# showlab/EgoVLP

Measured on AMD Instinct MI355X. Metric: clip-pairs/sec (whole node), 4f/224^2 ViT-B + 32-tok text, B=32/GPU, train step (fwd+gather+EgoNCE+bwd+AdamW), higher is better.
Workload: dtype fp16 (every Linear and both attentions of the video blocks, forward and backward) + bf16 (patch embedding, text tower, heads) MFMA operands, fp32 accumulate

## Files before the change

egovlp_amd/csrc/block.hip:

```cpp
#include <hip/hip_runtime.h>

#include <algorithm>

#include "layer_call.h"

namespace {

struct FwdLayout {
  int64_t n3_hi, n3_lo, mean3, rstd3, qkvt_hi, qkvt_lo, at_hi, at_lo, lse_t, work_t;
  int64_t tr, n1_hi, n1_lo, mean1, rstd1, qkvs_hi, qkvs_lo, as_hi, as_lo, lse_s, work_s;
  int64_t sr, n2_hi, n2_lo, mean2, rstd2, h_hi, h_lo, z;
  int64_t n3_bf, n1_bf, n2_bf, h_bf;
  int64_t n1c, mean1c, rstd1c, qc, oc, n2c, hc;
  int64_t total;
};

struct Geo {
  int64_t M, S, D, Hd;
  int P, Pb;
};

inline bool is_train(const egv_block_geom& g) { return (g.train & 1) != 0; }
inline bool is_tail(const egv_block_geom& g) { return (g.train & 2) != 0; }

// ... 277 lines not shown
  if (!gp || !pp || !iop || !geom_ok(*gp) || !(gp->train & 1)) return EGV_ERR_ARG;
  const egv_block_geom& g = *gp;
  const egv_block_params& p = *pp;
  const egv_block_bwd_io& io = *iop;
  if (!io.g_out || !io.x || !io.fwd_arena || !io.bwd_arena || !io.d_x || !io.dx_hi || !io.grads) return EGV_ERR_ARG;
  const bool tail = is_tail(g);
  if (tail && io.g_hi) return EGV_ERR_ARG;
  const Geo o = geo_of(g);
  const int Pb = o.Pb;
  const FwdLayout F = fwd_layout(g);
  const BwdLayout L = bwd_layout(g, io.wgrad_ksplit);
  int64_t goff[18], gtot;
  grad_layout(g, goff, gtot);
  const int32_t M = (int32_t)o.M, D = (int32_t)o.D, Hd = (int32_t)o.Hd;
  for (int i = 0; i < (tail ? 3 : 6); ++i)
    if (!p.wt_hi[i] || (Pb == 3 && !p.wt_lo[i])) return EGV_ERR_ARG;
  if (Pb == 3 && (!io.dx_lo || (io.g_hi && !io.g_lo))) return EGV_ERR_ARG;
  const bool h16 = Pb == 4;
  constexpr float A1_INV = 1.0f / (1.0f - 0.015625f);
  const char* FA = (const char*)io.fwd_arena;
  char* A = (char*)io.bwd_arena;
  hipStream_t main_s = (hipStream_t)stream;
  const bool x2 = o.P == 2 && !h16;
  const egv_bf16 *n3_hi, *n3_lo, *at_hi, *at_lo, *n1_hi, *n1_lo, *as_hi, *as_lo, *n2_hi, *n2_lo, *h_hi, *h_lo, *qt_hi, *qt_lo, *qs_hi, *qs_lo;
  saved_planes(FA, Pb, x2 ? F.n3_bf : F.n3_hi, F.n3_lo, n3_hi, n3_lo);
  saved_planes(FA, Pb, F.at_hi, F.at_lo, at_hi, at_lo);
  saved_planes(FA, Pb, x2 ? F.n1_bf : F.n1_hi, F.n1_lo, n1_hi, n1_lo);
  saved_planes(FA, Pb, F.as_hi, F.as_lo, as_hi, as_lo);
  saved_planes(FA, Pb, x2 ? F.n2_bf : F.n2_hi, F.n2_lo, n2_hi, n2_lo);
  saved_planes(FA, Pb, x2 ? F.h_bf : F.h_hi, F.h_lo, h_hi, h_lo);
  saved_planes(FA, Pb, F.qkvt_hi, F.qkvt_lo, qt_hi, qt_lo);
  saved_planes(FA, Pb, F.qkvs_hi, F.qkvs_lo, qs_hi, qs_lo);
  const bool proj1 = (g.f16_single & 8) != 0;
  const egv_bf16 *as_lo_f = (proj1 || h16) ? nullptr : at<egv_bf16>(FA, F.as_lo), *at_lo_f = (proj1 || h16) ? nullptr : at<egv_bf16>(FA, F.at_lo);
  const int afmt = h16 ? (proj1 ? 3 : 2) : (proj1 ? 1 : 0);
  const int amode = (afmt << 1) | (h16 ? 8 | 16 : 0);
  const float walpha[6] = {h16 && !(g.f16_single & 4) ? A1_INV : 1.0f, h16 && !proj1 ? A1_INV : 1.0f, h16 && !(g.f16_single & 4) ? A1_INV : 1.0f,
                           h16 && !proj1 ? A1_INV : 1.0f, h16 && !(g.f16_single & 1) ? A1_INV : 1.0f, h16 && !(g.f16_single & 2) ? A1_INV : 1.0f};
  const int Pg = Pb;
  const float *tr = at<float>(FA, F.tr), *sr = at<float>(FA, F.sr);
  float* grads = io.grads;

  bool defer_reduce = true;
  for (int i = 1; i < 6; ++i) defer_reduce = defer_reduce && io.side_stream[i] == io.side_stream[0];
#ifdef EGV_NO_MULTI_REDUCE
  defer_reduce = false;
#endif
  auto wgrad = [&](int i, const egv_bf16* dy_hi, const egv_bf16* dy_lo, int64_t lddy, const egv_bf16* x_hi, const egv_bf16* x_lo,
                   int64_t ldx, int64_t row0 = 0, int64_t rows = 0) -> int {
    int64_t N, K;
    wshape(o, i, N, K);
    if (rows) N = rows;
    hipStream_t s = main_s;
    if (io.side_stream[i]) {
      s = (hipStream_t)io.side_stream[i];
      if (hipEventRecord((hipEvent_t)io.side_event[i], main_s) != hipSuccess) return EGV_ERR_LAUNCH;
      if (hipStreamWaitEvent(s, (hipEvent_t)io.side_event[i], 0) != hipSuccess) return EGV_ERR_LAUNCH;
    }
    egv_gemm_desc d = tn_desc(dy_hi, dy_lo, lddy, x_hi, x_lo, ldx, N, K, M, Pg, grads + goff[i] + row0 * K, grads + goff[6 + i] + row0, io.wgrad_ksplit[i],
                              at<float>(A, L.partial[i]), g.grid_cap);
    d.alpha = walpha[i];
    if (defer_reduce && d.ksplit > 1) d.accumulate = 2;
    return egv_gemm_nt(&d, s);
  };

  auto ln_in = [&](egv_gemm_desc& d, float* buf) {
    if (h16) { d.out_hi = (egv_bf16*)buf; d.ldoh = D; d.out_fmt = 4; }
    else { d.out_f32 = buf; d.ldo = D; }
  };
  const int ln_fmt = h16 ? 3 : 0;
  float* d_sr = at<float>(A, L.d_sr);
  float* d_n1 = at<float>(A, L.d_n1);
  if (tail) {
    const float *w_q = (const float*)p.w_hi[2], *w_proj = (const float*)p.w_hi[3], *w_fc1 = (const float*)p.w_hi[4],
                *w_fc2 = (const float*)p.w_hi[5];
    if (!w_q || !w_proj || !w_fc1 || !w_fc2) return EGV_ERR_ARG;
    const int32_t B = g.B;
    const int64_t ldc = o.S * o.D;
    const float* G = io.g_out;
    const float *n1c = at<float>(FA, F.n1c), *qc = at<float>(FA, F.qc), *oc = at<float>(FA, F.oc), *n2c = at<float>(FA, F.n2c),
                *hc = at<float>(FA, F.hc);
    float *dzc = at<float>(A, L.dzc), *dn2c = at<float>(A, L.dn2c), *dsrc = at<float>(A, L.dsrc), *doc = at<float>(A, L.doc),
          *dqc = at<float>(A, L.dqc), *lw = at<float>(A, L.lin_work);
    EGV_TRY(egv_cls_linear_dgrad(G, D, w_fc2, Hd, B, D, Hd, at<float>(FA, F.z), dzc, Hd, 0, lw, stream));
    EGV_TRY(egv_cls_linear_wgrad(G, D, hc, Hd, B, D, Hd, grads + goff[5], Hd, grads + goff[11], stream));
    EGV_TRY(egv_cls_linear_dgrad(dzc, Hd, w_fc1, D, B, Hd, D, nullptr, dn2c, D, 0, lw, stream));
    EGV_TRY(egv_cls_linear_wgrad(dzc, Hd, n2c, D, B, Hd, D, grads + goff[4], D, grads + goff[10], stream));
    EGV_TRY(egv_layernorm_bwd_partial(dn2c, nullptr, nullptr, D, sr, D, p.n2w, at<float>(FA, F.mean2), at<float>(FA, F.rstd2), B, D, G, nullptr,
                                      dsrc, D, nullptr, nullptr, 0, grads + goff[16], grads + goff[17], at<float>(A, L.ln_work[0]), stream));
    EGV_TRY(egv_cls_linear_wgrad(dsrc, D, oc, D, B, D, D, grads + goff[3], D, grads + goff[9], stream));
    EGV_TRY(egv_cls_linear_dgrad(dsrc, D, w_proj, D, B, D, D, nullptr, doc, D, 0, lw, stream));
    uint16_t *dkv_hi = (uint16_t*)at<egv_bf16>(A, L.dqkvs_hi), *dkv_lo = (uint16_t*)at<egv_bf16>(A, L.dqkvs_lo);
    const uint16_t *kv_hi = (const uint16_t*)at<egv_bf16>(FA, F.qkvs_hi), *kv_lo = (const uint16_t*)at<egv_bf16>(FA, F.qkvs_lo);
    EGV_TRY(egv_cls_attn_bwd(qc, D, kv_hi, kv_lo, kv_hi + D, kv_lo ? kv_lo + D : nullptr, 2 * D, h16 ? 1 : 0, oc, doc, at<float>(FA, F.lse_s), B,
                             (int32_t)o.S, g.H, dqc, dkv_hi, dkv_lo, dkv_hi + D, dkv_lo ? dkv_lo + D : nullptr, 2 * D, h16 ? 1 : 0, stream));
    EGV_TRY(egv_cls_linear_wgrad(dqc, D, n1c, D, B, D, D, grads + goff[2], D, grads + goff[8], stream));
    EGV_TRY(wgrad(2, (const egv_bf16*)dkv_hi, (const egv_bf16*)dkv_lo, 2 * D, n1_hi, n1_lo, D, D, 2 * D));
    {
      egv_gemm_desc d = nt_desc((const egv_bf16*)dkv_hi, (const egv_bf16*)dkv_lo, 2 * D, p.wt_hi[2] + D, p.wt_lo[2] ? p.wt_lo[2] + D : nullptr,
                                p.ldwt[2], M, D, 2 * D, Pg, g.grid_cap);
      ln_in(d, d_n1);
      EGV_TRY(egv_gemm_nt(&d, stream));
    }
    EGV_TRY(egv_cls_linear_dgrad(dqc, D, w_q, D, B, D, D, nullptr, d_n1, ldc, h16 ? 2 : 1, lw, stream));
  } else {
    const egv_bf16 *g_hi = io.g_hi, *g_lo = Pb == 3 ? io.g_lo : nullptr;
    if (!g_hi) {
      egv_bf16 *gh = at<egv_bf16>(A, L.g_hi), *gl = at<egv_bf16>(A, L.g_lo);
      if (h16) EGV_TRY(egv_f16x2_encode(io.g_out, D, M, D, gh, nullptr, nullptr, D, 2, stream));
      else EGV_TRY(egv_split_f32(io.g_out, D, M, D, gh, gl, D, nullptr, nullptr, 0, nullptr, stream));
      g_hi = gh; g_lo = gl;
    }
    egv_bf16 *dz_hi = at<egv_bf16>(A, L.dz_hi), *dz_lo = at<egv_bf16>(A, L.dz_lo);
    {
      egv_gemm_desc d = nt_desc(g_hi, g_lo, D, p.wt_hi[5], p.wt_lo[5], p.ldwt[5], M, Hd, D, Pg, g.grid_cap);
      d.act = EGV_ACT_GELU_BWD; d.aux_in = at<float>(FA, F.z); d.ldaux = Hd; d.aux_bf16 = g.z_bf16 ? (h16 ? 3 : 2) : 0;
      d.out_hi = dz_hi; d.out_lo = dz_lo; d.ldoh = Hd;
      if (h16) d.out_fmt = 4;
      EGV_TRY(egv_gemm_nt(&d, stream));
    }
    EGV_TRY(wgrad(5, g_hi, g_lo, D, h_hi, h_lo, Hd));
    EGV_TRY(wgrad(4, dz_hi, dz_lo, Hd, n2_hi, n2_lo, D));
    float* d_n2 = at<float>(A, L.d_n2);
    {
      egv_gemm_desc d = nt_desc(dz_hi, dz_lo, Hd, p.wt_hi[4], p.wt_lo[4], p.ldwt[4], M, D, Hd, Pg, g.grid_cap);
      ln_in(d, d_n2);
      EGV_TRY(egv_gemm_nt(&d, stream));
    }
    egv_bf16 *dsr_hi = at<egv_bf16>(A, L.dsr_hi), *dsr_lo = at<egv_bf16>(A, L.dsr_lo);
    EGV_TRY(egv_layernorm_bwd_partial(h16 ? nullptr : d_n2, h16 ? (const egv_bf16*)d_n2 : nullptr, nullptr, D, sr, D, p.n2w, at<float>(FA, F.mean2),
                              at<float>(FA, F.rstd2), M, D, io.g_out, nullptr,
                              d_sr, D, dsr_hi, dsr_lo, ln_fmt, grads + goff[16], grads + goff[17], at<float>(A, L.ln_work[0]), stream));
    EGV_TRY(wgrad(3, dsr_hi, dsr_lo, D, as_hi, as_lo, D));
    egv_bf16 *das_hi = at<egv_bf16>(A, L.das_hi), *das_lo = at<egv_bf16>(A, L.das_lo);
    {
      egv_gemm_desc d = nt_desc(dsr_hi, dsr_lo, D, p.wt_hi[3], p.wt_lo[3], p.ldwt[3], M, D, D, Pg, g.grid_cap);
      d.out_hi = das_hi; d.out_lo = das_lo; d.ldoh = D;
      if (h16) d.out_fmt = 4;
      EGV_TRY(egv_gemm_nt(&d, stream));
    }
    egv_bf16 *dqs_hi = at<egv_bf16>(A, L.dqkvs_hi), *dqs_lo = at<egv_bf16>(A, L.dqkvs_lo);
    EGV_TRY(egv_divided_attn_bwd(qs_hi, qs_lo, as_hi, as_lo_f, das_hi, das_lo, at<float>(FA, F.lse_s), g.B, g.T, g.n, g.H, 0 | amode, h16 ? 1 : Pb, dqs_hi, dqs_lo,
                                 at<float>(A, L.attn_work), stream));
    EGV_TRY(wgrad(2, dqs_hi, dqs_lo, 3 * D, n1_hi, n1_lo, D));
    {
      egv_gemm_desc d = nt_desc(dqs_hi, dqs_lo, 3 * D, p.wt_hi[2], p.wt_lo[2], p.ldwt[2], M, D, 3 * D, Pg, g.grid_cap);
      ln_in(d, d_n1);
      EGV_TRY(egv_gemm_nt(&d, stream));
    }
  }
  float* d_tr = at<float>(A, L.d_tr);
  egv_bf16 *dtr_hi = at<egv_bf16>(A, L.dtr_hi), *dtr_lo = at<egv_bf16>(A, L.dtr_lo);
  EGV_TRY(egv_layernorm_bwd_partial(h16 ? nullptr : d_n1, h16 ? (const egv_bf16*)d_n1 : nullptr, nullptr, D, tr, D, p.n1w, at<float>(FA, F.mean1),
                            at<float>(FA, F.rstd1), M, D, nullptr, nullptr,
                            d_tr, D, dtr_hi, dtr_lo, ln_fmt, grads + goff[14], grads + goff[15], at<float>(A, L.ln_work[1]), stream));
  if (tail) EGV_TRY(egv_cls_rows_add(d_tr, o.S * o.D, at<float>(A, L.dsrc), D, g.B, D, stream));
  EGV_TRY(wgrad(1, dtr_hi, dtr_lo, D, at_hi, at_lo, D));
  egv_bf16 *dat_hi = at<egv_bf16>(A, L.dat_hi), *dat_lo = at<egv_bf16>(A, L.dat_lo);
  {
    egv_gemm_desc d = nt_desc(dtr_hi, dtr_lo, D, p.wt_hi[1], p.wt_lo[1], p.ldwt[1], M, D, D, Pg, g.grid_cap);
    d.out_hi = dat_hi; d.out_lo = dat_lo; d.ldoh = D;
    if (h16) d.out_fmt = 4;
    EGV_TRY(egv_gemm_nt(&d, stream));
  }
  egv_bf16 *dqt_hi = at<egv_bf16>(A, L.dqkvt_hi), *dqt_lo = at<egv_bf16>(A, L.dqkvt_lo);
  EGV_TRY(egv_divided_attn_bwd(qt_hi, qt_lo, at_hi, at_lo_f, dat_hi, dat_lo, at<float>(FA, F.lse_t), g.B, g.T, g.n, g.H, 1 | amode, h16 ? 1 : Pb, dqt_hi, dqt_lo,
                               at<float>(A, L.attn_work), stream));
  EGV_TRY(wgrad(0, dqt_hi, dqt_lo, 3 * D, n3_hi, n3_lo, D));
  float* d_n3 = at<float>(A, L.d_n3);
  {
    egv_gemm_desc d = nt_desc(dqt_hi, dqt_lo, 3 * D, p.wt_hi[0], p.wt_lo[0], p.ldwt[0], M, D, 3 * D, Pg, g.grid_cap);
    ln_in(d, d_n3);
    EGV_TRY(egv_gemm_nt(&d, stream));
  }
  EGV_TRY(egv_layernorm_bwd_partial(h16 ? nullptr : d_n3, h16 ? (const egv_bf16*)d_n3 : nullptr, nullptr, D, io.x, D, p.n3w, at<float>(FA, F.mean3),
                            at<float>(FA, F.rstd3), M, D, d_tr, d_sr,
                            io.d_x, D, io.dx_hi, Pb == 3 ? io.dx_lo : nullptr, ln_fmt, grads + goff[12], grads + goff[13],
                            at<float>(A, L.ln_work[2]), stream));
  if (defer_reduce) {
// ... 28 lines not shown
```

egovlp_amd/csrc/cls_tail.hip:

```cpp
#include <hip/hip_runtime.h>

#include "egovlp_hip.h"
#include "f16x2.h"

namespace {

constexpr int LIN_CT = 4;
constexpr int LIN_RT = 8;
constexpr int DG_NS = 64;
constexpr int DG_RT = 8;

__global__ __launch_bounds__(256) void cls_linear_fwd_kernel(const float* __restrict__ x, long ldx, const float* __restrict__ W, long ldw,
                                                             const float* __restrict__ bias, int R, int N, int K, int act,
                                                             float* __restrict__ z_out, const float* __restrict__ res, long ldr,
                                                             float* __restrict__ y, long ldy) {
  __shared__ float red[4][LIN_CT * LIN_RT];
  const int n0 = blockIdx.x * LIN_CT, r0 = blockIdx.y * LIN_RT;
  const int lane = threadIdx.x & 63, wave = threadIdx.x >> 6;
  float acc[LIN_CT][LIN_RT];
#pragma unroll
  for (int c = 0; c < LIN_CT; ++c)
#pragma unroll
    for (int r = 0; r < LIN_RT; ++r) acc[c][r] = 0.f;
  const int nr = min(LIN_RT, R - r0);
  for (int k4 = threadIdx.x; k4 < K / 4; k4 += 256) {
    f32x4_t w[LIN_CT];
#pragma unroll
    for (int c = 0; c < LIN_CT; ++c) w[c] = *(const f32x4_t*)(W + (long)(n0 + c) * ldw + k4 * 4);
#pragma unroll
    for (int r = 0; r < LIN_RT; ++r) {
      if (r < nr) {
        const f32x4_t xv = *(const f32x4_t*)(x + (long)(r0 + r) * ldx + k4 * 4);
#pragma unroll
        for (int c = 0; c < LIN_CT; ++c) acc[c][r] += w[c][0] * xv[0] + w[c][1] * xv[1] + w[c][2] * xv[2] + w[c][3] * xv[3];
      }
    }
  }
#pragma unroll
  for (int c = 0; c < LIN_CT; ++c)
#pragma unroll
    for (int r = 0; r < LIN_RT; ++r) {
      const float s = wave_sum(acc[c][r]);
      if (lane == 0) red[wave][c * LIN_RT + r] = s;
    }
  __syncthreads();
  if (threadIdx.x < LIN_CT * LIN_RT) {
    const int c = threadIdx.x / LIN_RT, r = threadIdx.x % LIN_RT;
    if (r < nr) {
      const int n = n0 + c;
      const long row = r0 + r;
      float v = red[0][threadIdx.x] + red[1][threadIdx.x] + red[2][threadIdx.x] + red[3][threadIdx.x];
      if (bias) v += bias[n];
      if (z_out) z_out[row * N + n] = v;
      if (act == EGV_ACT_GELU) v = gelu_f(v);
      if (res) v += res[row * ldr + n];
      y[row * ldy + n] = v;
    }
  }
}

__global__ __launch_bounds__(256) void cls_linear_dgrad_kernel(const float* __restrict__ dy, long lddy, const float* __restrict__ W, long ldw,
                                                               int R, int N, int K, float* __restrict__ partial) {
  __shared__ float dys[DG_RT][DG_NS];
  const int n0 = blockIdx.x * DG_NS, r0 = blockIdx.y * DG_RT;
  const int nn = min(DG_NS, N - n0), nr = min(DG_RT, R - r0);
  for (int i = threadIdx.x; i < DG_RT * DG_NS; i += 256) {
    const int r = i / DG_NS, n = i % DG_NS;
    dys[r][n] = (r < nr && n < nn) ? dy[(long)(r0 + r) * lddy + n0 + n] : 0.f;
  }
  __syncthreads();
  for (int k4 = blockIdx.z * 256 + threadIdx.x; k4 < K / 4; k4 += gridDim.z * 256) {
    f32x4_t acc[DG_RT];
#pragma unroll
    for (int r = 0; r < DG_RT; ++r) acc[r] = (f32x4_t){0.f, 0.f, 0.f, 0.f};
    for (int n = 0; n < nn; ++n) {
      const f32x4_t w = *(const f32x4_t*)(W + (long)(n0 + n) * ldw + k4 * 4);
#pragma unroll
      for (int r = 0; r < DG_RT; ++r) acc[r] += dys[r][n] * w;
    }
#pragma unroll
    for (int r = 0; r < DG_RT; ++r)
      if (r < nr) *(f32x4_t*)(partial + ((long)blockIdx.x * R + r0 + r) * K + k4 * 4) = acc[r];
  }
}

__global__ __launch_bounds__(256) void cls_linear_dgrad_finish_kernel(const float* __restrict__ partial, int slabs, int R, int K,
                                                                      const float* __restrict__ z, void* __restrict__ dx, long lddx, int mode) {
  const long i = (long)blockIdx.x * 256 + threadIdx.x;
  if (i >= (long)R * K) return;
  const int r = (int)(i / K), k = (int)(i % K);
  float v = 0.f;
  for (int s = 0; s < slabs; ++s) v += partial[(long)s * R * K + i];
  if (z) v *= gelu_grad_f(z[i]);
  if (mode == 2) {
    _Float16* p = (_Float16*)dx + (long)r * lddx + k;
    *p = (_Float16)((float)*p + v);
  } else {
    float* p = (float*)dx + (long)r * lddx + k;
    *p = mode == 1 ? *p + v : v;
  }
}

__global__ __launch_bounds__(256) void cls_linear_wgrad_kernel(const float* __restrict__ dy, long lddy, const float* __restrict__ x, long ldx,
                                                               int R, int N, int K, float* __restrict__ dW, long lddw, float* __restrict__ db) {
  const int n0 = blockIdx.x * 4;
  const int k4 = blockIdx.y * 256 + threadIdx.x;
  if (db && blockIdx.y == 0 && threadIdx.x < 4) {
    float s = 0.f;
    for (int r = 0; r < R; ++r) s += dy[(long)r * lddy + n0 + threadIdx.x];
    db[n0 + threadIdx.x] = s;
  }
  if (k4 >= K / 4) return;
  f32x4_t acc[4];
#pragma unroll
  for (int j = 0; j < 4; ++j) acc[j] = (f32x4_t){0.f, 0.f, 0.f, 0.f};
  for (int r = 0; r < R; ++r) {
    const f32x4_t xv = *(const f32x4_t*)(x + (long)r * ldx + k4 * 4);
    const f32x4_t g = *(const f32x4_t*)(dy + (long)r * lddy + n0);
#pragma unroll
    for (int j = 0; j < 4; ++j) acc[j] += g[j] * xv;
  }
#pragma unroll
  for (int j = 0; j < 4; ++j) *(f32x4_t*)(dW + (long)(n0 + j) * lddw + k4 * 4) = acc[j];
}

__global__ __launch_bounds__(256) void cls_rows_add_kernel(float* __restrict__ dst, long lddst, const float* __restrict__ src, long ldsrc, int R,
                                                           int cols) {
  const long i = (long)blockIdx.x * 256 + threadIdx.x;
  if (i >= (long)R * cols) return;
  const int r = (int)(i / cols), c = (int)(i % cols);
  dst[(long)r * lddst + c] += src[(long)r * ldsrc + c];
}


template <int FMT>
__device__ __forceinline__ void load8(const uint16_t* hi, const uint16_t* lo, long off, float (&v)[8]) {
  const u32x4_t a = *(const u32x4_t*)(hi + off);
  u32x4_t b = (u32x4_t){0u, 0u, 0u, 0u};
  if (lo) b = *(const u32x4_t*)(lo + off);
// ... 74 lines not shown
template <int FMT, int DFMT>
__global__ __launch_bounds__(256) void cls_attn_bwd_kernel(const float* __restrict__ q, long ldq, const uint16_t* __restrict__ k_hi,
                                                           const uint16_t* __restrict__ k_lo, const uint16_t* __restrict__ v_hi,
                                                           const uint16_t* __restrict__ v_lo, long ldkv, const float* __restrict__ out,
                                                           const float* __restrict__ d_out, const float* __restrict__ lse, int S, int H,
                                                           float* __restrict__ dq, uint16_t* __restrict__ dk_hi, uint16_t* __restrict__ dk_lo,
                                                           uint16_t* __restrict__ dv_hi, uint16_t* __restrict__ dv_lo, long lddkv) {
  __shared__ float sdq[32][64];
  const int b = blockIdx.x / H, h = blockIdx.x % H;
  const int sub = threadIdx.x & 7, grp = threadIdx.x >> 3;
  const long D = (long)H * 64;
  float qv[8], dov[8], dqa[8];
  float dl = 0.f;
#pragma unroll
  for (int e = 0; e < 8; ++e) {
    const long c = (long)b * D + h * 64 + sub * 8 + e;
    qv[e] = q[(long)b * ldq + h * 64 + sub * 8 + e] * ATTN_SCALE;
    dov[e] = d_out[c];
    dl += dov[e] * out[c];
    dqa[e] = 0.f;
  }
  const float delta = group8_sum(dl);
  const float L = lse[b * H + h];
  for (int j = grp; j < S; j += 32) {
    const long off = ((long)b * S + j) * ldkv + h * 64 + sub * 8;
    float kv[8], vv[8];
    load8<FMT>(k_hi, k_lo, off, kv);
    load8<FMT>(v_hi, v_lo, off, vv);
    float s = 0.f, dp = 0.f;
#pragma unroll
    for (int e = 0; e < 8; ++e) {
      s += qv[e] * kv[e];
      dp += dov[e] * vv[e];
    }
    s = group8_sum(s);
    dp = group8_sum(dp);
    const float p = __expf(s - L);
    const float ds = p * (dp - delta);
    float dk[8], dv[8];
#pragma unroll
    for (int e = 0; e < 8; ++e) {
      dk[e] = ds * qv[e];
      dv[e] = p * dov[e];
      dqa[e] += ds * kv[e];
    }
    const long doff = ((long)b * S + j) * lddkv + h * 64 + sub * 8;
    if (DFMT == 1) {
      *(u32x4_t*)(dk_hi + doff) = f16_grad_piece8(dk);
      *(u32x4_t*)(dv_hi + doff) = f16_grad_piece8(dv);
    } else {
      u32x4_t kh, kl, vh, vl;
#pragma unroll
      for (int e = 0; e < 4; ++e) {
        uint32_t a, b2, c, d;
        split_bf16x2(dk[2 * e], dk[2 * e + 1], a, b2);
        split_bf16x2(dv[2 * e], dv[2 * e + 1], c, d);
        kh[e] = a; kl[e] = b2; vh[e] = c; vl[e] = d;
      }
      *(u32x4_t*)(dk_hi + doff) = kh;
      *(u32x4_t*)(dv_hi + doff) = vh;
      if (dk_lo) *(u32x4_t*)(dk_lo + doff) = kl;
      if (dv_lo) *(u32x4_t*)(dv_lo + doff) = vl;
    }
  }
#pragma unroll
  for (int e = 0; e < 8; ++e) sdq[grp][sub * 8 + e] = dqa[e];
  __syncthreads();
  if (threadIdx.x < 64) {
    float s = 0.f;
    for (int g = 0; g < 32; ++g) s += sdq[g][threadIdx.x];
    dq[(long)b * D + h * 64 + threadIdx.x] = s * ATTN_SCALE;
  }
}

bool aligned16(const void* p) { return ((uintptr_t)p & 15) == 0; }

}

extern "C" int egv_cls_linear_fwd(const float* x, int64_t ldx, const float* W, int64_t ldw, const float* bias, int32_t R, int32_t N,
                                  int32_t K, int32_t act, float* z_out, const float* residual, int64_t ldr, float* y, int64_t ldy,
                                  void* stream) {
  if (!x || !W || !y || R <= 0 || N <= 0 || K <= 0 || N % 4 || K % 4 || ldx % 4 || ldw % 4 || ldx < K || ldw < K || ldy < N) return EGV_ERR_ARG;
  if ((act != EGV_ACT_NONE && act != EGV_ACT_GELU) || (residual && ldr < N) || !aligned16(x) || !aligned16(W)) return EGV_ERR_ARG;
  EGV_LAUNCH(cls_linear_fwd_kernel, dim3(N / LIN_CT, (R + LIN_RT - 1) / LIN_RT), dim3(256), 0, (hipStream_t)stream, x, ldx, W, ldw, bias, R, N,
             K, act, z_out, residual, ldr, y, ldy);
  EGV_CHECK_LAUNCH();
  return EGV_OK;
}

extern "C" int64_t egv_cls_linear_work_floats(int32_t R, int32_t N, int32_t K) {
  if (R <= 0 || N <= 0 || K <= 0) return -1;
  return (int64_t)((N + DG_NS - 1) / DG_NS) * R * K;
}

extern "C" int egv_cls_linear_dgrad(const float* dy, int64_t lddy, const float* W, int64_t ldw, int32_t R, int32_t N, int32_t K, const float* z,
                                    void* dx, int64_t lddx, int32_t dx_mode, float* work, void* stream) {
  if (!dy || !W || !dx || !work || R <= 0 || N <= 0 || K <= 0 || K % 4 || ldw % 4 || ldw < K || lddy < N || lddx < K) return EGV_ERR_ARG;
  if (dx_mode < 0 || dx_mode > 2 || !aligned16(W) || !aligned16(work)) return EGV_ERR_ARG;
  const int slabs = (N + DG_NS - 1) / DG_NS;
  const int kz = (K / 4 + 255) / 256;
  EGV_LAUNCH(cls_linear_dgrad_kernel, dim3(slabs, (R + DG_RT - 1) / DG_RT, kz), dim3(256), 0, (hipStream_t)stream, dy, lddy, W, ldw, R, N, K, work);
  EGV_CHECK_LAUNCH();
  const int64_t tot = (int64_t)R * K;
  EGV_LAUNCH(cls_linear_dgrad_finish_kernel, dim3((unsigned)((tot + 255) / 256)), dim3(256), 0, (hipStream_t)stream, work, slabs, R, K, z, dx,
             lddx, dx_mode);
  EGV_CHECK_LAUNCH();
  return EGV_OK;
}

extern "C" int egv_cls_linear_wgrad(const float* dy, int64_t lddy, const float* x, int64_t ldx, int32_t R, int32_t N, int32_t K, float* dW,
                                    int64_t lddw, float* db, void* stream) {
  if (!dy || !x || !dW || R <= 0 || N <= 0 || K <= 0 || N % 4 || K % 4 || lddy % 4 || ldx % 4 || lddw % 4 || lddy < N || ldx < K || lddw < K)
    return EGV_ERR_ARG;
  if (!aligned16(dy) || !aligned16(x) || !aligned16(dW)) return EGV_ERR_ARG;
  EGV_LAUNCH(cls_linear_wgrad_kernel, dim3(N / 4, (K / 4 + 255) / 256), dim3(256), 0, (hipStream_t)stream, dy, lddy, x, ldx, R, N, K, dW, lddw,
             db);
  EGV_CHECK_LAUNCH();
  return EGV_OK;
}

extern "C" int egv_cls_rows_add(float* dst, int64_t lddst, const float* src, int64_t ldsrc, int32_t R, int32_t cols, void* stream) {
  if (!dst || !src || R <= 0 || cols <= 0 || lddst < cols || ldsrc < cols) return EGV_ERR_ARG;
  const int64_t tot = (int64_t)R * cols;
  EGV_LAUNCH(cls_rows_add_kernel, dim3((unsigned)((tot + 255) / 256)), dim3(256), 0, (hipStream_t)stream, dst, lddst, src, ldsrc, R, cols);
  EGV_CHECK_LAUNCH();
  return EGV_OK;
}

extern "C" int egv_cls_attn_fwd(const float* q, int64_t ldq, const uint16_t* k_hi, const uint16_t* k_lo, const uint16_t* v_hi,
                                const uint16_t* v_lo, int64_t ldkv, int32_t kv_fmt, int32_t B, int32_t S, int32_t H, float* out, int64_t ldo,
                                float* lse, void* stream) {
  if (!q || !k_hi || !v_hi || !out || !lse || B <= 0 || S <= 0 || H <= 0 || (kv_fmt != 0 && kv_fmt != 1)) return EGV_ERR_ARG;
  if (ldkv % 8 || ldkv < (int64_t)H * 64 || ldq < (int64_t)H * 64 || ldo < (int64_t)H * 64 || (k_lo == nullptr) != (v_lo == nullptr))
    return EGV_ERR_ARG;
  if (!aligned16(k_hi) || !aligned16(v_hi) || !aligned16(k_lo) || !aligned16(v_lo)) return EGV_ERR_ARG;
  if (kv_fmt == 1)
    EGV_LAUNCH(cls_attn_fwd_kernel<1>, dim3(B * H), dim3(256), 0, (hipStream_t)stream, q, ldq, k_hi, k_lo, v_hi, v_lo, ldkv, S, H, out, ldo, lse);
  else
    EGV_LAUNCH(cls_attn_fwd_kernel<0>, dim3(B * H), dim3(256), 0, (hipStream_t)stream, q, ldq, k_hi, k_lo, v_hi, v_lo, ldkv, S, H, out, ldo, lse);
  EGV_CHECK_LAUNCH();
  return EGV_OK;
}

extern "C" int egv_cls_attn_bwd(const float* q, int64_t ldq, const uint16_t* k_hi, const uint16_t* k_lo, const uint16_t* v_hi,
                                const uint16_t* v_lo, int64_t ldkv, int32_t kv_fmt, const float* out, const float* d_out, const float* lse,
                                int32_t B, int32_t S, int32_t H, float* dq, uint16_t* dk_hi, uint16_t* dk_lo, uint16_t* dv_hi, uint16_t* dv_lo,
                                int64_t lddkv, int32_t d_fmt, void* stream) {
  if (!q || !k_hi || !v_hi || !out || !d_out || !lse || !dq || !dk_hi || !dv_hi || B <= 0 || S <= 0 || H <= 0) return EGV_ERR_ARG;
  if ((kv_fmt != 0 && kv_fmt != 1) || (d_fmt != 0 && d_fmt != 1) || (d_fmt == 1 && (dk_lo || dv_lo))) return EGV_ERR_ARG;
  if (ldkv % 8 || lddkv % 8 || ldkv < (int64_t)H * 64 || lddkv < (int64_t)H * 64 || ldq < (int64_t)H * 64) return EGV_ERR_ARG;
  if ((k_lo == nullptr) != (v_lo == nullptr) || (dk_lo == nullptr) != (dv_lo == nullptr)) return EGV_ERR_ARG;
  if (!aligned16(k_hi) || !aligned16(v_hi) || !aligned16(k_lo) || !aligned16(v_lo) || !aligned16(dk_hi) || !aligned16(dv_hi) || !aligned16(dk_lo) ||
      !aligned16(dv_lo))
    return EGV_ERR_ARG;
  hipStream_t s = (hipStream_t)stream;
#define EGV_CLS_BWD(F, DF)                                                                                                              \
  EGV_LAUNCH((cls_attn_bwd_kernel<F, DF>), dim3(B * H), dim3(256), 0, s, q, ldq, k_hi, k_lo, v_hi, v_lo, ldkv, out, d_out, lse, S, H, dq, dk_hi, \
             dk_lo, dv_hi, dv_lo, lddkv)
  if (kv_fmt == 1 && d_fmt == 1) EGV_CLS_BWD(1, 1);
  else if (kv_fmt == 1) EGV_CLS_BWD(1, 0);
  else if (d_fmt == 1) EGV_CLS_BWD(0, 1);
  else EGV_CLS_BWD(0, 0);
#undef EGV_CLS_BWD
  EGV_CHECK_LAUNCH();
  return EGV_OK;
}
```

egovlp_amd/model/video_transformer.py:

```python
from __future__ import annotations

import ctypes as C
from functools import partial

import torch
from torch import nn

from .. import _lib, ops
from .._lib import BlockBwdIO, BlockGeom, BlockParams
from ..ops import ACT_GELU, ACT_GELU_BWD, ExecContext
from .layer_common import (PLANE_HANDOFF, _attach_grad_planes, _lin_bwd, _take_grad_planes, bwd_arena_bytes,
                           gelu_grad_16bit, grad_views, layer_sizes, need_fwd_arena, param_struct)


def f16x2_block_ok(M, D, Hd, train):
    if not (ops.f16x2_gemm_ok(M, 3 * D, D) and ops.f16x2_gemm_ok(M, Hd, D) and ops.f16x2_gemm_ok(M, D, Hd)):
        return False
    return not train or ops.uses_big_gemm(M, Hd, D, 1)


class _SpaceTimeBlockFn(torch.autograd.Function):

    @staticmethod
    def forward(ctx, x, geom, ec: ExecContext,
# ... 163 lines not shown
def _block_params(wc, ln, biases, weights, need_t, x2=False, proj_x2=False, t16=False):
    fmts = [("f16x2" if (proj_x2 and i in (1, 3)) else _X2_FMTS[i]) if x2 else "bf16" for i in range(6)]
    pls = [wc.get(w, need_t=need_t, fmt=fmts[i], t_fmt="f16" if t16 else "bf16") for i, w in enumerate(weights)]
    return param_struct(wc, BlockParams, (id(weights[0]), need_t, x2, proj_x2, t16), need_t, ln, biases, pls)


class _SpaceTimeBlockCFn(torch.autograd.Function):

    @staticmethod
    def forward(ctx, x, geom, ec: ExecContext,
                n3w, n3b, tqkv_w, tqkv_b, tproj_w, tproj_b,
                n1w, n1b, sqkv_w, sqkv_b, sproj_w, sproj_b,
                n2w, n2b, fc1_w, fc1_b, fc2_w, fc2_b):
        B, T, n, H, eps = geom[:5]
        S = 1 + T * n
        D = x.shape[-1]
        M = B * S
        Hd = fc1_w.shape[0]
        P, Pb = ec.fwd_passes, ec.bwd_passes
        single = (geom[5] if len(geom) > 5 else 0) if P == 2 else 0
        dev = x.device
        x2 = x.contiguous().view(M, D)
        save = any(ctx.needs_input_grad)
        train = ec.forward_is_train(ctx)
        tail = len(geom) > 7 and bool(geom[7])
        key = (B, T, n, H, D, Hd, P, Pb, train, gelu_grad_16bit(ec, M, Hd, D, P), single)
        g = _block_geom(*key, eps, ec.gemm_grid, tail)
        ent = layer_sizes("egv_block", key + (tail,), g, 18)
        arena = torch.empty(ent[0], dtype=torch.uint8, device=dev)
        out = torch.empty((B if tail else M, D), dtype=torch.float32, device=dev)
        ln = (n3w, n3b, n1w, n1b, n2w, n2b)
        biases = (tqkv_b, tproj_b, sqkv_b, sproj_b, fc1_b, fc2_b)
        weights = (tqkv_w, tproj_w, sqkv_w, sproj_w, fc1_w, fc2_w)
        prm = _block_params(ec.wc, ln, biases, weights, need_t=False, x2=P == 2, proj_x2=bool(single & 8) or Pb == 4)
        if tail:
            prm = _tail_params(prm, weights, need_t=False)
        _lib.check(_lib.lib().egv_block_fwd(C.byref(g), C.byref(prm), x2.data_ptr(), out.data_ptr(), arena.data_ptr(), ops._stream(x2)),
                   "egv_block_fwd")
        if save:
            ctx.key, ctx.eps, ctx.ec, ctx.arena, ctx.sizes, ctx.tail = key, eps, ec, arena, ent, tail
            ctx.save_for_backward(x2, *ln, *biases, *weights)
        return out if tail else out.view(B, S, D)

    @staticmethod
    def backward(ctx, g_out):
        saved = ctx.saved_tensors
        x2, ln, biases, weights = saved[0], saved[1:7], saved[7:13], saved[13:19]
        need_fwd_arena(ctx.arena, "block")
        B, T, n, H, D, Hd, P, Pb, train, z_bf16, single = ctx.key
        ec = ctx.ec
        ec.poll_backward()
        Pb_now = ec.bwd_passes
        if Pb_now != Pb:
            raise RuntimeError("the backward precision changed between this block's forward and its backward")
        S = 1 + T * n
        M = B * S
        dev = x2.device
        tail = ctx.tail
        G = g_out.contiguous().view(B if tail else M, D)
        g_pl = None if tail else _take_grad_planes(g_out, M, D, Pb)
        g_hi, g_lo = (g_pl.hi.data_ptr(), ops._p(g_pl.lo)) if g_pl is not None else (None, None)
        shapes = [(w.shape[0], w[0].numel()) for w in weights]
        order = (5, 4, 3, 2, 1, 0)
        side_ok = ec.wgrad_side_stream and not ec.on_text_stream()
        use = [side_ok and weights[i].grad is None for i in range(6)]
        deal = ec.assign_side_streams([float(M) * shapes[i][0] * shapes[i][1] for i in order if use[i]]) if any(use) else []
        streams, events = [None] * 6, [None] * 6
        it = iter(deal)
        for i in order:
            if use[i]:
                streams[i], events[i] = next(it)
        if tail:
            shapes[2] = (2 * D, D)
        ks = [1 if tail and i > 2 else ops.wgrad_ksplit(shapes[i][0], shapes[i][1], M, ec, use[i]) for i in range(6)]
        g = _block_geom(*ctx.key, ctx.eps, ec.gemm_grid, tail)
        ks6 = (C.c_int32 * 6)(*ks)
        barena = torch.empty(bwd_arena_bytes("egv_block", (ctx.key, tail, tuple(ks)), g, ks6), dtype=torch.uint8, device=dev)
        _, goff, gtot = ctx.sizes
        grads = torch.empty(gtot, dtype=torch.float32, device=dev)
        d_x = torch.empty((M, D), dtype=torch.float32, device=dev)
        dx_pl = ops.empty_planes_f16x2(M, D, dev, single=True) if Pb == 4 else ops.empty_planes(M, D, Pb, dev)
        used = {s_ for s_ in streams if s_ is not None}
        if used:
            ec.hold_until_join(ctx.arena, barena, grads, *((g_pl.hi, g_pl.lo) if g_pl is not None else ()))
        prm = _block_params(ec.wc, ln, biases, weights, need_t=True, x2=P == 2, proj_x2=bool(single & 8) or Pb == 4, t16=Pb == 4)
        if tail:
            prm = _tail_params(prm, weights, need_t=True)
        P6 = C.c_void_p * 6
        io = BlockBwdIO(G.data_ptr(), g_hi, g_lo, x2.data_ptr(), ctx.arena.data_ptr(), barena.data_ptr(),
                        d_x.data_ptr(), dx_pl.hi.data_ptr(), ops._p(dx_pl.lo), grads.data_ptr(),
                        P6(*[s_.cuda_stream if s_ is not None else None for s_ in streams]),
                        P6(*[e.cuda_event if e is not None else None for e in events]), ks6)
        _lib.check(_lib.lib().egv_block_bwd(C.byref(g), C.byref(prm), C.byref(io), ops._stream(x2)), "egv_block_bwd")
        ctx.arena = None

        parts = grad_views(grads, goff, gtot)
        dW = [parts[i].view(weights[i].shape) for i in range(6)]
        db = parts[6:12]
        dln = parts[12:18]
        return (_attach_grad_planes(d_x.view(B, S, D), Pb, dx_pl), None, None,
                dln[0], dln[1], dW[0], db[0], dW[1], db[1],
                dln[2], dln[3], dW[2], db[2], dW[3], db[3],
                dln[4], dln[5], dW[4], db[4], dW[5], db[5])


class _PatchTokensFn(torch.autograd.Function):

    @staticmethod
    def forward(ctx, video, geom, ec, proj_w, proj_b, cls_token, pos_embed, temporal_embed):
        B, T, n, P_, D, T_model = geom[:6]
        Pp = ec.fwd_passes_split
        wc = ec.wc
        mean, std = geom[6] if len(geom) > 6 else (ops.IMAGENET_MEAN, ops.IMAGENET_STD)
        aug = geom[7] if len(geom) > 7 else None
        ev = geom[8] if len(geom) > 8 else None
        keep = geom[9] if len(geom) > 9 else None
        if ev is not None:
            a = ops.patch_gather_eval(video.contiguous(), ev[2], T, P_, Pp, ev[0], ev[1], mean, std)
        else:
            if aug is not None and len(aug) > 2:
                a = ops.patch_gather(video.contiguous(), P_, Pp, mean, std, aug=aug[:2], keep=keep, color=aug[2])
            else:
                a = ops.patch_gather(video.contiguous(), P_, Pp, mean, std, aug=aug, keep=keep)
        K = proj_w[0].numel()
        if a.cols == K:
            w_pl = wc.get(proj_w, need_t=False)[0]
        else:
            w_pl = ops.split_f32(torch.nn.functional.pad(proj_w.detach().reshape(D, K), (0, a.cols - K)), Pp)[0]
        pe = torch.empty((a.rows, D), dtype=torch.float32, device=video.device)
        ops.gemm_nt(a, w_pl, passes=Pp, bias=proj_b, out_f32=pe, ec=ec)
        x = ops.assemble_tokens(pe, cls_token, pos_embed, temporal_embed, B, T, n, D, keep=keep)
        ctx.geom, ctx.a, ctx.Pp, ctx.ec = geom[:9], a, Pp, ec
        ctx.save_for_backward(*(() if keep is None else (keep,)))
        ctx.wshape, ctx.proj_w = proj_w.shape, proj_w
        return x

    @staticmethod
    def backward(ctx, dx):
        B, T, n, P_, D, T_model = ctx.geom[:6]
        ec = ctx.ec
        Pb = 1 if ec.bwd_passes == 4 else ec.bwd_passes
        ec.poll_backward()
        keep = ctx.saved_tensors[0] if ctx.saved_tensors else None
        d_pe, d_cls, d_pos, d_tmp = ops.assemble_tokens_bwd(dx.contiguous(), B, T, n, D, T_model, keep=keep)
        K = ctx.wshape[1] * ctx.wshape[2] * ctx.wshape[3]
        _, d_w, d_b = _lin_bwd(d_pe, ctx.a, None, Pb, need_dx=False, params=(ctx.proj_w,), ec=ec, allow_side=(ctx.a.cols == K))
        if d_w.shape[1] != K:
            d_w = d_w[:, :K].contiguous()
        return None, None, None, d_w.view(ctx.wshape), d_b, d_cls, d_pos, d_tmp


class _ClsNormFn(torch.autograd.Function):

    @staticmethod
    def forward(ctx, x, w, b, eps, ec):
        xc = x.contiguous()
        if x.dim() == 2:
            _, y, mean, rstd, _ = ops.layernorm_fwd(xc, w, b, eps, 1, want_f32=True, want_planes=False)
        else:
            B, S, D = x.shape
            _, y, mean, rstd, _ = ops.layernorm_fwd(xc.view(B * S, D), w, b, eps, 1, want_f32=True, want_planes=False,
                                                    rows=B, ldx=S * D)
        ctx.save_for_backward(xc, w, mean, rstd)
        ctx.ec = ec
        return y

    @staticmethod
# ... 289 lines not shown
```

Before: 1050.

## Overlap CLS-tail weight-grad kernels on side streams and restructure CLS linear forward

In the tail block's backward, the CLS-token weight-gradient kernels now go to the per-weight side streams behind an event on the main stream, so they can overlap with the dependent dgrad chain. The gradient input G is held until the streams join so it stays alive. The CLS linear forward kernel changes from one block per (column tile, 8-row tile) to one block per column tile that loops over 32-row chunks. It also prefetches the next weight vector and replaces the per-value wave reductions with a shuffle reduce-scatter. This cuts launch blocks and shuffle work for small R, at the cost of fewer blocks in flight and more registers.

```diff
diff --git a/egovlp_amd/csrc/block.hip b/egovlp_amd/csrc/block.hip
--- a/egovlp_amd/csrc/block.hip
+++ b/egovlp_amd/csrc/block.hip
@@ -383,19 +383,28 @@
                 *hc = at<float>(FA, F.hc);
     float *dzc = at<float>(A, L.dzc), *dn2c = at<float>(A, L.dn2c), *dsrc = at<float>(A, L.dsrc), *doc = at<float>(A, L.doc),
           *dqc = at<float>(A, L.dqc), *lw = at<float>(A, L.lin_work);
+    auto cls_wgrad = [&](int i, const float* dy, int64_t lddy, const float* xr, int64_t ldx, int32_t N, int32_t K) -> int {
+      void* s = stream;
+      if (io.side_stream[i]) {
+        s = io.side_stream[i];
+        if (hipEventRecord((hipEvent_t)io.side_event[i], main_s) != hipSuccess) return EGV_ERR_LAUNCH;
+        if (hipStreamWaitEvent((hipStream_t)s, (hipEvent_t)io.side_event[i], 0) != hipSuccess) return EGV_ERR_LAUNCH;
+      }
+      return egv_cls_linear_wgrad(dy, lddy, xr, ldx, B, N, K, grads + goff[i], K, grads + goff[6 + i], s);
+    };
     EGV_TRY(egv_cls_linear_dgrad(G, D, w_fc2, Hd, B, D, Hd, at<float>(FA, F.z), dzc, Hd, 0, lw, stream));
-    EGV_TRY(egv_cls_linear_wgrad(G, D, hc, Hd, B, D, Hd, grads + goff[5], Hd, grads + goff[11], stream));
+    EGV_TRY(cls_wgrad(5, G, D, hc, Hd, D, Hd));
     EGV_TRY(egv_cls_linear_dgrad(dzc, Hd, w_fc1, D, B, Hd, D, nullptr, dn2c, D, 0, lw, stream));
-    EGV_TRY(egv_cls_linear_wgrad(dzc, Hd, n2c, D, B, Hd, D, grads + goff[4], D, grads + goff[10], stream));
+    EGV_TRY(cls_wgrad(4, dzc, Hd, n2c, D, Hd, D));
     EGV_TRY(egv_layernorm_bwd_partial(dn2c, nullptr, nullptr, D, sr, D, p.n2w, at<float>(FA, F.mean2), at<float>(FA, F.rstd2), B, D, G, nullptr,
                                       dsrc, D, nullptr, nullptr, 0, grads + goff[16], grads + goff[17], at<float>(A, L.ln_work[0]), stream));
-    EGV_TRY(egv_cls_linear_wgrad(dsrc, D, oc, D, B, D, D, grads + goff[3], D, grads + goff[9], stream));
+    EGV_TRY(cls_wgrad(3, dsrc, D, oc, D, D, D));
     EGV_TRY(egv_cls_linear_dgrad(dsrc, D, w_proj, D, B, D, D, nullptr, doc, D, 0, lw, stream));
     uint16_t *dkv_hi = (uint16_t*)at<egv_bf16>(A, L.dqkvs_hi), *dkv_lo = (uint16_t*)at<egv_bf16>(A, L.dqkvs_lo);
     const uint16_t *kv_hi = (const uint16_t*)at<egv_bf16>(FA, F.qkvs_hi), *kv_lo = (const uint16_t*)at<egv_bf16>(FA, F.qkvs_lo);
     EGV_TRY(egv_cls_attn_bwd(qc, D, kv_hi, kv_lo, kv_hi + D, kv_lo ? kv_lo + D : nullptr, 2 * D, h16 ? 1 : 0, oc, doc, at<float>(FA, F.lse_s), B,
                              (int32_t)o.S, g.H, dqc, dkv_hi, dkv_lo, dkv_hi + D, dkv_lo ? dkv_lo + D : nullptr, 2 * D, h16 ? 1 : 0, stream));
-    EGV_TRY(egv_cls_linear_wgrad(dqc, D, n1c, D, B, D, D, grads + goff[2], D, grads + goff[8], stream));
+    EGV_TRY(cls_wgrad(2, dqc, D, n1c, D, D, D));
     EGV_TRY(wgrad(2, (const egv_bf16*)dkv_hi, (const egv_bf16*)dkv_lo, 2 * D, n1_hi, n1_lo, D, D, 2 * D));
     {
       egv_gemm_desc d = nt_desc((const egv_bf16*)dkv_hi, (const egv_bf16*)dkv_lo, 2 * D, p.wt_hi[2] + D, p.wt_lo[2] ? p.wt_lo[2] + D : nullptr,
diff --git a/egovlp_amd/csrc/cls_tail.hip b/egovlp_amd/csrc/cls_tail.hip
--- a/egovlp_amd/csrc/cls_tail.hip
+++ b/egovlp_amd/csrc/cls_tail.hip
@@ -6,55 +6,82 @@
 namespace {
 
 constexpr int LIN_CT = 4;
-constexpr int LIN_RT = 8;
+constexpr int LIN_RT = 32;
 constexpr int DG_NS = 64;
 constexpr int DG_RT = 8;
 
-__global__ __launch_bounds__(256) void cls_linear_fwd_kernel(const float* __restrict__ x, long ldx, const float* __restrict__ W, long ldw,
+__device__ __forceinline__ float dot4_add(float acc, const f32x4_t w, const f32x4_t x, bool odd) {
+  float t = odd ? __builtin_fmaf(w[1], x[1], w[0] * x[0]) : __builtin_fmaf(w[0], x[0], w[1] * x[1]);
+  t = __builtin_fmaf(w[2], x[2], t);
+  t = __builtin_fmaf(w[3], x[3], t);
+  return acc + t;
+}
+
+template <int NV, int O = 32>
+__device__ __forceinline__ void wave_sum_scatter(float (&v)[NV], int lane) {
+  constexpr int half = NV / 2;
+  const bool up = (lane & O) != 0;
+#pragma unroll
+  for (int i = 0; i < half; ++i) {
+    const float send = up ? v[i] : v[i + half];
+    const float keep = up ? v[i + half] : v[i];
+    v[i] = keep + __shfl_xor(send, O, 64);
+  }
+  if constexpr (O > 1) wave_sum_scatter<half, O / 2>(reinterpret_cast<float (&)[half]>(v), lane);
+}
+
+__global__ __launch_bounds__(256, 2) void cls_linear_fwd_kernel(const float* __restrict__ x, long ldx, const float* __restrict__ W, long ldw,
                                                              const float* __restrict__ bias, int R, int N, int K, int act,
                                                              float* __restrict__ z_out, const float* __restrict__ res, long ldr,
                                                              float* __restrict__ y, long ldy) {
-  __shared__ float red[4][LIN_CT * LIN_RT];
-  const int n0 = blockIdx.x * LIN_CT, r0 = blockIdx.y * LIN_RT;
+  constexpr int NV = LIN_CT * LIN_RT;
+  __shared__ float red[4][NV];
+  const int n0 = blockIdx.x * LIN_CT;
   const int lane = threadIdx.x & 63, wave = threadIdx.x >> 6;
-  float acc[LIN_CT][LIN_RT];
-#pragma unroll
-  for (int c = 0; c < LIN_CT; ++c)
-#pragma unroll
-    for (int r = 0; r < LIN_RT; ++r) acc[c][r] = 0.f;
-  const int nr = min(LIN_RT, R - r0);
-  for (int k4 = threadIdx.x; k4 < K / 4; k4 += 256) {
-    f32x4_t w[LIN_CT];
-#pragma unroll
-    for (int c = 0; c < LIN_CT; ++c) w[c] = *(const f32x4_t*)(W + (long)(n0 + c) * ldw + k4 * 4);
-#pragma unroll
-    for (int r = 0; r < LIN_RT; ++r) {
+  const int K4 = K / 4;
+  for (int r0 = 0; r0 < R; r0 += LIN_RT) {
+    const int nr = min(LIN_RT, R - r0);
+    float acc[NV];
+#pragma unroll
+    for (int i = 0; i < NV; ++i) acc[i] = 0.f;
+    f32x4_t wn[LIN_CT];
+    if ((int)threadIdx.x < K4) {
+#pragma unroll
+      for (int c = 0; c < LIN_CT; ++c) wn[c] = *(const f32x4_t*)(W + (long)(n0 + c) * ldw + threadIdx.x * 4);
+    }
+    for (int k4 = threadIdx.x; k4 < K4; k4 += 256) {
+      f32x4_t w[LIN_CT];
+#pragma unroll
+      for (int c = 0; c < LIN_CT; ++c) w[c] = wn[c];
+      if (k4 + 256 < K4) {
+#pragma unroll
+        for (int c = 0; c < LIN_CT; ++c) wn[c] = *(const f32x4_t*)(W + (long)(n0 + c) * ldw + (k4 + 256) * 4);
+      }
+#pragma unroll
+      for (int r = 0; r < LIN_RT; ++r) {
+        const f32x4_t xv = *(const f32x4_t*)(x + (long)(r0 + min(r, nr - 1)) * ldx + k4 * 4);
+#pragma unroll
+        for (int c = 0; c < LIN_CT; ++c) acc[c * LIN_RT + r] = dot4_add(acc[c * LIN_RT + r], w[c], xv, (c & 1) != 0);
+      }
+    }
+    wave_sum_scatter<NV>(acc, lane);
+    if (r0) __syncthreads();
+    const int slot = lane * (NV / 64);
+#pragma unroll
+    for (int i = 0; i < NV / 64; ++i) red[wave][slot + i] = acc[i];
+    __syncthreads();
+    if (threadIdx.x < NV) {
+      const int c = threadIdx.x / LIN_RT, r = threadIdx.x % LIN_RT;
       if (r < nr) {
-        const f32x4_t xv = *(const f32x4_t*)(x + (long)(r0 + r) * ldx + k4 * 4);
-#pragma unroll
-        for (int c = 0; c < LIN_CT; ++c) acc[c][r] += w[c][0] * xv[0] + w[c][1] * xv[1] + w[c][2] * xv[2] + w[c][3] * xv[3];
+        const int n = n0 + c;
+        const long row = r0 + r;
+        float v = red[0][threadIdx.x] + red[1][threadIdx.x] + red[2][threadIdx.x] + red[3][threadIdx.x];
+        if (bias) v += bias[n];
+        if (z_out) z_out[row * N + n] = v;
+        if (act == EGV_ACT_GELU) v = gelu_f(v);
+        if (res) v += res[row * ldr + n];
+        y[row * ldy + n] = v;
       }
-    }
-  }
-#pragma unroll
-  for (int c = 0; c < LIN_CT; ++c)
-#pragma unroll
-    for (int r = 0; r < LIN_RT; ++r) {
-      const float s = wave_sum(acc[c][r]);
-      if (lane == 0) red[wave][c * LIN_RT + r] = s;
-    }
-  __syncthreads();
-  if (threadIdx.x < LIN_CT * LIN_RT) {
-    const int c = threadIdx.x / LIN_RT, r = threadIdx.x % LIN_RT;
-    if (r < nr) {
-      const int n = n0 + c;
-      const long row = r0 + r;
-      float v = red[0][threadIdx.x] + red[1][threadIdx.x] + red[2][threadIdx.x] + red[3][threadIdx.x];
-      if (bias) v += bias[n];
-      if (z_out) z_out[row * N + n] = v;
-      if (act == EGV_ACT_GELU) v = gelu_f(v);
-      if (res) v += res[row * ldr + n];
-      y[row * ldy + n] = v;
     }
   }
 }
@@ -295,7 +322,7 @@
                                   void* stream) {
   if (!x || !W || !y || R <= 0 || N <= 0 || K <= 0 || N % 4 || K % 4 || ldx % 4 || ldw % 4 || ldx < K || ldw < K || ldy < N) return EGV_ERR_ARG;
   if ((act != EGV_ACT_NONE && act != EGV_ACT_GELU) || (residual && ldr < N) || !aligned16(x) || !aligned16(W)) return EGV_ERR_ARG;
-  EGV_LAUNCH(cls_linear_fwd_kernel, dim3(N / LIN_CT, (R + LIN_RT - 1) / LIN_RT), dim3(256), 0, (hipStream_t)stream, x, ldx, W, ldw, bias, R, N,
+  EGV_LAUNCH(cls_linear_fwd_kernel, dim3(N / LIN_CT), dim3(256), 0, (hipStream_t)stream, x, ldx, W, ldw, bias, R, N,
              K, act, z_out, residual, ldr, y, ldy);
   EGV_CHECK_LAUNCH();
   return EGV_OK;
diff --git a/egovlp_amd/model/video_transformer.py b/egovlp_amd/model/video_transformer.py
--- a/egovlp_amd/model/video_transformer.py
+++ b/egovlp_amd/model/video_transformer.py
@@ -269,7 +269,7 @@
         dx_pl = ops.empty_planes_f16x2(M, D, dev, single=True) if Pb == 4 else ops.empty_planes(M, D, Pb, dev)
         used = {s_ for s_ in streams if s_ is not None}
         if used:
-            ec.hold_until_join(ctx.arena, barena, grads, *((g_pl.hi, g_pl.lo) if g_pl is not None else ()))
+            ec.hold_until_join(ctx.arena, barena, grads, *((g_pl.hi, g_pl.lo) if g_pl is not None else ()), *((G,) if tail else ()))
         prm = _block_params(ec.wc, ln, biases, weights, need_t=True, x2=P == 2, proj_x2=bool(single & 8) or Pb == 4, t16=Pb == 4)
         if tail:
             prm = _tail_params(prm, weights, need_t=True)
```

New measurement: 1050. About the same (-0.0%).
